# zijieli-Jlee/Temporal-Pointcloud-Upsampling-GAN

Hardware: AMD Instinct MI355X
Metric: GAN train-steps/sec (G+D) on 4096-pt x3-frame clips (higher is better)
Workload: dtype bf16; 1 GPU; cfg2: 4096-pt x3-frame fluid clips, full G+D adversarial step (SRNet(3,128) + FluidTempoDis(3) + FluidSpatialDis, Adam), all-keep mask regime, gate open, even iteration; batch 8 per GPU; per_gpu_batch=8, global_batch=8, parallelism=dp1, step_mode=hipgraph (1 graph per step)

## Files before the change

include/tpgan_ops.h:

```cpp
#ifndef TPGAN_OPS_H
#define TPGAN_OPS_H

#include <stddef.h>
#include <stdint.h>

#ifdef __cplusplus
extern "C" {
#endif

typedef enum {
    TPG_OK = 0,
    TPG_ERR_ARG = -1,
    TPG_ERR_LAUNCH = -2,
    TPG_ERR_UNSUPPORTED = -3
} tpg_status;

#define TPG_MAX_K 64

const char *tpg_version(void);
const char *tpg_target_arch(void);

int tpg_knn_f32(const float *p1, const float *p2, const int64_t *len1,
                const int64_t *len2, int B, int P1, int P2, int D, int K,
                float r2, float *dist, int64_t *idx, void *stream);

int tpg_knn_grid_f32(const float *p1, const float *p2, const int64_t *len1, const int64_t *len2, int B,
                     int P1, int P2, int K, float *dist, int64_t *idx, void *ws, void *stream);

int tpg_knn_mfma_f32(const float *p1, const float *p2, const int64_t *len1,
                     const int64_t *len2, int B, int P1, int P2, int D, int K,
                     float *dist, int64_t *idx, int redo, void *stream);

size_t tpg_frnn_grid_workspace_bytes(int B, int P2);
int tpg_frnn_grid_f32(const float *p1, const float *p2, const int64_t *len1, const int64_t *len2, int B, int P1,
                      int P2, int K, float r, float *dist, int64_t *idx, void *ws, void *stream);

int tpg_chamfer_fwd_f32(const float *src, const float *tgt, int B, int N, int M,
                        float *d1, int64_t *i1, float *d2, int64_t *i2,
                        void *stream);
size_t tpg_chamfer_bwd_workspace_bytes(int B, int N, int M);
int tpg_chamfer_bwd_f32(const float *src, const float *tgt, int B, int N, int M,
                        const int64_t *i1, const int64_t *i2, const float *g1,
                        const float *g2, float *gsrc, float *gtgt, void *ws, void *stream);

int tpg_fps_f32(const float *xyz, int B, int N, int m, float *temp, int32_t *idx,
                void *stream);

int tpg_fps_prefix_f32(const float *xyz, int B, int N, int m, float *temp, int32_t *idx,
                       const int32_t *prefix_in, int32_t *prefix_out, void *stream);

int tpg_fps_start_f32(const float *xyz, const int32_t *start, int skip_origin, int B, int N, int m,
                      float *temp, int32_t *idx, void *stream);

int tpg_gather_fwd_f32(const float *feat, const int32_t *idx, int B, int C, int N,
                       int S, float *out, void *stream);
int tpg_gather_bwd_f32(const float *gout, const int32_t *idx, int B, int C, int N,
                       int S, float *gfeat, void *stream);

int tpg_gather_rows_fwd_f32(const float *rows, const int32_t *idx, int B, int N, int S, int C, float *out, void *stream);
int tpg_gather_rows_bwd_f32(const float *gout, const int32_t *idx, int B, int N, int S, int C, float *grows,
                            void *stream);

int tpg_ball_query_f32(const float *xyz, const float *new_xyz, int B, int N, int S,
                       float radius, int nsample, int32_t *idx, void *stream);

int tpg_group_fwd_f32(const float *feat, const int32_t *idx, int B, int C, int N,
                      int S, int K, float *out, void *stream);
int tpg_group_bwd_f32(const float *gout, const int32_t *idx, int B, int C, int N,
                      int S, int K, float *gfeat, void *stream);

int tpg_three_nn_f32(const float *unknown, const float *known, int B, int n, int m,
                     float *dist2, int32_t *idx, void *stream);
int tpg_three_interp_fwd_f32(const float *feat, const int32_t *idx, const float *w,
                             int B, int C, int m, int n, float *out, void *stream);
int tpg_three_interp_bwd_f32(const float *gout, const int32_t *idx, const float *w,
                             int B, int C, int m, int n, float *gfeat,
                             void *stream);

typedef enum { TPG_DTYPE_F32 = 0, TPG_DTYPE_BF16 = 1 } tpg_dtype;

int tpg_rowcombine_fwd(const void *U, const void *QE, const int32_t *idx, int mode, int dtype_in,
                       int dtype_out, int B, int N, int S, int K, int C, float slope, void *out,
                       void *stream);

int tpg_invert_index(const int32_t *idx, int B, int N, int SK, int32_t *offs, int32_t *list,
                     int32_t *tmp, void *stream);

int tpg_rowcombine_bwd(const void *gout, const int32_t *idx, const int32_t *offs, const int32_t *list,
                       const void *E, int mode, int dtype_in, int dtype_out, int B, int N, int S, int K,
                       int C, float slope, void *gU, void *gQE, void *stream);

int tpg_rowcombine_edge_fwd(const void *Y, const int32_t *idx, int dtype_in, int dtype_out, int B, int N, int K, int C,
                            float slope_a, float slope_e, void *out, void *stream);
int tpg_rowcombine_edge_bwd(const void *gout, const int32_t *idx, const int32_t *offs, const int32_t *list,
                            const void *Y, int dtype_in, int dtype_out, int B, int N, int K, int C, float slope_a,
                            float slope_e, void *gY, void *stream);

int tpg_head_bn_act_fwd(const float *h, int B, int C, const float *gamma, const float *beta, float *running_mean,
                        float *running_var, long long *num_batches_tracked, float momentum, float eps, float slope,
                        const float *mask, float *y, float *mean, float *rstd, void *stream);
int tpg_head_bn_act_bwd(const float *gy, const float *h, const float *mean, const float *rstd, const float *gamma,
                        const float *beta, float slope, const float *mask, int B, int C, float *dh, float *dgamma,
                        float *dbeta, void *stream);

#define TPG_BN_PHASE_ALL 0
#define TPG_BN_PHASE_STATS 1
#define TPG_BN_PHASE_APPLY 2
size_t tpg_rowbn_workspace_bytes(int C, int nseg);
int tpg_rowbn_fwd(const void *x, int dtype_in, long long P, int K, int C, float eps, float momentum,
                  int training, float *running_mean, float *running_var, long long *num_batches_tracked,
                  const float *mean_shift, const float *gamma, const float *beta, float slope, float *mean,
                  float *rstd, void *y,
                  int dtype_out, uint8_t *argmax, void *ws, int nseg, int phase, void *stream);
int tpg_rowbn_bwd(const void *gy, int dtype_g, const void *x, int dtype_in, const uint8_t *argmax,
// ... 170 lines not shown
```

temporal-pointcloud-upsampling-gan_amd/_lib.py:

```python
import ctypes as C
import os

_HERE = os.path.dirname(os.path.abspath(__file__))
LIB_PATH = os.environ.get("TPGAN_HIP_LIBRARY") or os.path.join(_HERE, "csrc", "libtpgan_hip.so")

_P = C.c_void_p
_I = C.c_int
_F = C.c_float
_L = C.c_longlong

SIGNATURES = {
    "tpg_knn_f32": [_P, _P, _P, _P, _I, _I, _I, _I, _I, _F, _P, _P, _P],
    "tpg_knn_mfma_f32": [_P, _P, _P, _P, _I, _I, _I, _I, _I, _P, _P, _I, _P],
    "tpg_knn_grid_f32": [_P, _P, _P, _P, _I, _I, _I, _I, _P, _P, _P, _P],
    "tpg_frnn_grid_f32": [_P, _P, _P, _P, _I, _I, _I, _I, _F, _P, _P, _P, _P],
    "tpg_chamfer_fwd_f32": [_P, _P, _I, _I, _I, _P, _P, _P, _P, _P],
    "tpg_chamfer_bwd_f32": [_P, _P, _I, _I, _I, _P, _P, _P, _P, _P, _P, _P, _P],
    "tpg_fps_f32": [_P, _I, _I, _I, _P, _P, _P],
    "tpg_fps_prefix_f32": [_P, _I, _I, _I, _P, _P, _P, _P, _P],
    "tpg_fps_start_f32": [_P, _P, _I, _I, _I, _I, _P, _P, _P],
    "tpg_gather_fwd_f32": [_P, _P, _I, _I, _I, _I, _P, _P],
    "tpg_gather_bwd_f32": [_P, _P, _I, _I, _I, _I, _P, _P],
    "tpg_ball_query_f32": [_P, _P, _I, _I, _I, _F, _I, _P, _P],
    "tpg_group_fwd_f32": [_P, _P, _I, _I, _I, _I, _I, _P, _P],
    "tpg_group_bwd_f32": [_P, _P, _I, _I, _I, _I, _I, _P, _P],
    "tpg_three_nn_f32": [_P, _P, _I, _I, _I, _P, _P, _P],
    "tpg_three_interp_fwd_f32": [_P, _P, _P, _I, _I, _I, _I, _P, _P],
    "tpg_three_interp_bwd_f32": [_P, _P, _P, _I, _I, _I, _I, _P, _P],
    "tpg_gather_rows_fwd_f32": [_P, _P, _I, _I, _I, _I, _P, _P],
    "tpg_gather_rows_bwd_f32": [_P, _P, _I, _I, _I, _I, _P, _P],
    "tpg_rowcombine_fwd": [_P, _P, _P, _I, _I, _I, _I, _I, _I, _I, _I, _F, _P, _P],
    "tpg_invert_index": [_P, _I, _I, _I, _P, _P, _P, _P],
    "tpg_rowcombine_bwd": [_P, _P, _P, _P, _P, _I, _I, _I, _I, _I, _I, _I, _I, _F, _P, _P, _P],
    "tpg_rowcombine_edge_fwd": [_P, _P, _I, _I, _I, _I, _I, _I, _F, _F, _P, _P],
    "tpg_rowcombine_edge_bwd": [_P, _P, _P, _P, _P, _I, _I, _I, _I, _I, _I, _F, _F, _P, _P],
    "tpg_head_bn_act_fwd": [_P, _I, _I, _P, _P, _P, _P, _P, _F, _F, _F, _P, _P, _P, _P, _P],
    "tpg_head_bn_act_bwd": [_P, _P, _P, _P, _P, _P, _F, _P, _I, _I, _P, _P, _P, _P],
    "tpg_rowbn_fwd": [_P, _I, _L, _I, _I, _F, _F, _I, _P, _P, _P, _P, _P, _P, _F, _P, _P, _P, _I, _P, _P, _I, _I, _P],
    "tpg_rowbn_bwd": [_P, _I, _P, _I, _P, _P, _I, _L, _I, _I, _I, _P, _P, _P, _P, _F, _P, _P, _P, _P, _I, _I, _P],
    "tpg_cubic_interp_f32": [_P, _P, _P, _I, _I, _I, _I, _F, _P, _P, _P, _P],
    "tpg_spectral_norm_fwd": [_P, _P, _P, _I, _I, _I, _F, _P, _P, _P],
    "tpg_spectral_norm_bwd": [_P, _P, _P, _P, _P, _I, _I, _P, _P],
    "tpg_spectral_norm_multi_fwd": [_P, _I, _I, _P, _I, _F, _P],
    "tpg_spectral_norm_multi_fwd_split": [_P, _P, _I, _I, _P, _P, _L, _F, _P],
    "tpg_spectral_norm_multi_bwd": [_P, _I, _I, _P, _P, _P, _P, _P],
    "tpg_rowbn_bwd_sums": [_P, _I, _P, _I, _P, _P, _I, _L, _I, _I, _I, _P, _P, _P, _P, _F, _P, _P, _P, _P, _I, _P],
    "tpg_rowbn_bwd_sums_consts": [_P, _I, _P, _I, _P, _P, _I, _L, _I, _I, _I, _P, _P, _P, _P, _F, _P, _P, _P, _P, _P, _P, _I, _P],
    "tpg_rowbn_stats_consts": [_P, _I, _L, _I, _F, _F, _P, _P, _P, _P, _P, _P, _P, _P, _P, _P, _I, _P],
    "tpg_mlp_consts": [_P, _P, _P, _P, _P, _I, _I, _P, _P, _P],
    "tpg_mlp_max_prep": [_P, _P, _P, _F, _L, _I, _I, _P, _P],
    "tpg_mlp_dgrad": [_P, _P, _P, _I, _P, _P, _P, _F, _P, _I, _L, _I, _I, _I, _I, _P, _P, _P, _P, _P, _P, _P],
    "tpg_mlp_wgrad": [_P, _P, _P, _I, _P, _P, _P, _F, _L, _I, _I, _I, _I, _P, _P, _P],
    "tpg_mlp_bn_bwd_apply": [_P, _P, _P, _P, _L, _I, _I, _P, _P],
    "tpg_mlp_bn_bwd_apply_rowsum": [_P, _P, _P, _P, _L, _I, _I, _I, _P, _P, _P],
    "tpg_small_tail_fwd": [_P, _I, _P, _P, _F, _F, _L, _I, _I, _I, _I, _P, _P, _P],
    "tpg_small_tail_bwd": [_P, _P, _P, _P, _I, _P, _P, _F, _F, _L, _I, _I, _I, _I, _P, _P, _P, _P, _P],
    "tpg_rowlinear_fwd": [_P, _I, _P, _P, _L, _I, _I, _I, _F, _P, _I, _P],
    "tpg_rowlinear_dgrad": [_P, _P, _I, _P, _L, _I, _I, _I, _F, _P, _I, _P],
    "tpg_rowlinear_wgrad": [_P, _I, _P, _P, _I, _L, _I, _I, _I, _F, _P, _P, _P, _P],
    "tpg_mlp_fwd": [_P, _L, _I, _I, _I, _P, _I, _F, _P, _I, _P, _F, _F, _P, _P, _P, _P, _P, _P, _P, _P, _P, _P, _P],
    "tpg_mlp_infer_fwd": [_P, _P, _P, _I, _I, _I, _I, _I, _I, _I, _I, _P, _P, _P, _P, _P, _P, _F, _F, _F, _P, _P],
    "tpg_context_expand_f32": [_P, _P, _P, _I, _I, _I, _I, _P, _P, _P, _P, _P],
    "tpg_radius_reduce_f32": [_P, _P, _P, _P, _I, _I, _I, _F, _I, _P, _P, _P, _P],
    "tpg_radius_reduce_exhaustive_f32": [_P, _P, _P, _P, _I, _I, _I, _F, _I, _P, _P, _P],
    "tpg_patch_select_f32": [_P, _L, _P, _P, _P, _I, _I, _P, _P, _P],
    "tpg_clip_gather_high_f32": [_P, _P, _L, _P, _P, _P, _I, _P, _P, _I, _I, _I, _P, _P, _P],
    "tpg_clip_gather_low_f32": [_P, _P, _P, _F, _P, _L, _P, _P, _I, _I, _I, _I, _P, _P, _P],
    "tpg_frame_subset": [_P, _P, _I, _I, _P, _P],
    "tpg_action_gather_f32": [_P, _L, _P, _P, _P, _P, _I, _I, _I, _I, _P, _P, _P],
    "tpg_replace_dummy_centres": [_P, _P, _P, _I, _I, _I, _I, _P, _P, _P, _P],
    "tpg_emd_init_f32": [_P, _I, _I, _I, _I, _P, _P, _P],
    "tpg_emd_rounds_f32": [_P, _I, _I, _F, _F, _I, _I, _I, _I, _I, _P, _P, _P],
    "tpg_emd_finish_f32": [_P, _I, _I, _P, _P, _P, _P, _P, _P],
    "tpg_gaussian_row_sums_f32": [_P, _P, _P, _P, _I, _I, _I, _F, _P, _P],
    "tpg_render_points_f32": [_P, _P, _P, _I, _I, _P, _I, _I, _I, _I, _F, _F, _P, _P, _P, _P, _P, _P],
    "tpg_render_spheres_f32": [_P, _P, _I, _I, _P, _I, _I, _I, _F, _P, _P, _P, _P],
    "tpg_surface_smooth_f32": [_P, _I, _I, _I, _I, _F, _P, _P],
    "tpg_surface_shade_f32": [_P, _P, _P, _I, _I, _P, _I, _I, _I, _F, _F, _P, _P, _P, _P, _P],
    "tpg_pbf_predict_f32": [_P, _P, _P, _P, _I, _I, _F, _F, _P, _P, _P, _P],
    "tpg_pbf_grid_f32": [_P, _P, _I, _I, _F, _P, _P],
    "tpg_pbf_lambda_f32": [_P, _P, _I, _I, _F, _F, _F, _P, _P, _P, _P],
    "tpg_pbf_dp_f32": [_P, _P, _P, _P, _I, _I, _F, _F, _F, _F, _F, _P, _P, _P, _P],
    "tpg_pbf_finish_f32": [_P, _P, _P, _I, _I, _F, _F, _F, _P, _P, _P, _P],
    "tpg_iso_count_f32": [_P, _I, _I, _I, _F, _P, _P, _P],
    "tpg_iso_emit_f32": [_P, _I, _I, _I, _P, _F, _F, _P, _L, _L, _P, _P, _P, _P],
}
SIZE_GETTERS = ("tpg_rowbn_workspace_bytes", "tpg_mlp_workspace_bytes", "tpg_context_expand_workspace_bytes",
                "tpg_emd_workspace_bytes", "tpg_pbf_workspace_bytes", "tpg_iso_workspace_bytes")
OTHER_GETTERS = ("tpg_spectral_norm_multi_stride", "tpg_spectral_norm_multi_bwd_scratch",
                 "tpg_mlp_wgrad_workspace_bytes", "tpg_frnn_grid_workspace_bytes", "tpg_small_tail_workspace_bytes",
                 "tpg_chamfer_bwd_workspace_bytes", "tpg_rowlinear_wgrad_workspace_bytes", "tpg_rowlinear_supported",
                 "tpg_spectral_norm_split_rows", "tpg_spectral_norm_split_max_cn", "tpg_spectral_norm_split_max_rows",
                 "tpg_patch_select_workspace_bytes", "tpg_patch_select_max_k", "tpg_mlp_infer_supported")
STRING_GETTERS = ("tpg_version", "tpg_target_arch")

STATUS = {0: "TPG_OK", -1: "TPG_ERR_ARG", -2: "TPG_ERR_LAUNCH", -3: "TPG_ERR_UNSUPPORTED"}
# ... 59 lines not shown
```

temporal-pointcloud-upsampling-gan_amd/csrc/knn.hip:

```cpp
#include <cstdlib>
#include <type_traits>

#include <hip/hip_bf16.h>

#include "invert_index.hpp"
#include "knn_select.hpp"
#include "tpg_common.hpp"

namespace {

constexpr int KNN_WAVES = 4;

template <int D_T>
__device__ __forceinline__ float knn_dist(const float *__restrict__ qs,
                                          const float *__restrict__ c, int D) {
    float acc = 0.0f;
    if constexpr (D_T == 3) {
        acc = tpg_sq3(qs[0], qs[1], qs[2], c[0], c[1], c[2]);
    } else if constexpr (D_T > 0) {
        static_assert(D_T % 4 == 0, "vector path needs D % 4 == 0");
        const float4 *c4 = reinterpret_cast<const float4 *>(c);
        const float4 *q4 = reinterpret_cast<const float4 *>(qs);
#pragma unroll
        for (int d = 0; d < D_T / 4; ++d) {
// ... 152 lines not shown
        if (i >= P1 || lane >= K) continue;
        const size_t o = ((size_t)b * P1 + i) * K + lane;
        if (i >= n1 || n2 <= 0 || best[qq] == TPG_KNN_INF) { dist[o] = pad_d; idx[o] = pad_i; }
        else { dist[o] = tpg_knn_key_dist(best[qq]); idx[o] = tpg_knn_key_idx(best[qq]); }
    }
}

template <int D_T>
__global__ __launch_bounds__(KNN_WAVES * 64) void knn_redo_kernel(
    const float *__restrict__ p1, const float *__restrict__ p2, const int64_t *__restrict__ len1,
    const int64_t *__restrict__ len2, int P1, int P2, int K, float *__restrict__ dist, int64_t *__restrict__ idx) {
    __shared__ __attribute__((aligned(16))) float qs[D_T];
    __shared__ tpg_u64 slots[KNN_WAVES * 64];
    __shared__ tpg_u64 lists[KNN_WAVES * 64];
    const int lane = threadIdx.x & 63;
    const int wave = __builtin_amdgcn_readfirstlane(threadIdx.x >> 6);
    const int b = blockIdx.y;
    const int n1 = len1 ? (int)len1[b] : P1;
    const int n2 = len2 ? min((int)len2[b], P2) : P2;
    const float *cbase = p2 + (size_t)b * P2 * D_T;
    for (int u = 0; u < KNN_WAVES; ++u) {
        const int i = blockIdx.x * KNN_WAVES + u;
        if (i >= P1) break;
        const size_t q = (size_t)b * P1 + i;
        if (idx[q * K] != KM_REDO_MARK) continue;
        __syncthreads();
        if (threadIdx.x < D_T) qs[threadIdx.x] = p1[q * D_T + threadIdx.x];
        __syncthreads();
        tpg_u64 best = TPG_KNN_INF, thr = TPG_KNN_INF;
        if (i < n1)
            for (int base = wave * 64; base < n2; base += KNN_WAVES * 64) {
                const int j = base + lane;
                const tpg_u64 key =
                    j < n2 ? tpg_knn_key(knn_dist<D_T>(qs, cbase + (size_t)j * D_T, D_T), j) : TPG_KNN_INF;
                tpg_knn_merge(best, thr, key, K, lane, slots + wave * 64);
            }
        lists[wave * 64 + lane] = lane < K ? best : TPG_KNN_INF;
        __syncthreads();
        if (wave == 0) {
            best = TPG_KNN_INF;
            thr = TPG_KNN_INF;
            for (int w = 0; w < KNN_WAVES; ++w) tpg_knn_merge(best, thr, lists[w * 64 + lane], K, lane, slots);
            if (lane < K) {
                if (best == TPG_KNN_INF) { dist[q * K + lane] = 0.0f; idx[q * K + lane] = 0; }
                else { dist[q * K + lane] = tpg_knn_key_dist(best); idx[q * K + lane] = tpg_knn_key_idx(best); }
            }
        }
    }
}

#include "knn_mfma.hpp"

#ifndef TPG_KNN_MFMA_MIN_POINTS
#define TPG_KNN_MFMA_MIN_POINTS 2048
#endif

template <int D_T, int M>
int knn_mfma_launch_m(const float *p1, const float *p2, const int64_t *len1, const int64_t *len2, int B, int P1, int P2,
                      int K, float *dist, int64_t *idx, bool redo, hipStream_t st) {
    if (!tpg_allow_dynamic_lds<&knn_mfma_kernel<D_T, M>>((int)km_smem_bytes<D_T>())) return TPG_ERR_LAUNCH;
    const int gx = (P1 + KM_Q - 1) / KM_Q;
    const long long total = (long long)gx * B;
    if (total > (1ll << 30)) return TPG_ERR_ARG;
    const unsigned grid = (unsigned)((total + 7) / 8 * 8);
    hipLaunchKernelGGL((knn_mfma_kernel<D_T, M>), dim3(grid), dim3(KM_WAVES * 64), km_smem_bytes<D_T>(), st, p1, p2, len1, len2,
                       P1, P2, K, gx, (int)total, dist, idx);
    TPG_RETURN_IF_LAUNCH_FAILED();
    if (redo) {
        const dim3 rg((unsigned)((P1 + KNN_WAVES - 1) / KNN_WAVES), (unsigned)B);
        hipLaunchKernelGGL((knn_redo_kernel<D_T>), rg, dim3(KNN_WAVES * 64), 0, st, p1, p2, len1, len2, P1, P2, K, dist, idx);
        TPG_RETURN_IF_LAUNCH_FAILED();
    }
    return TPG_OK;
}

template <int D_T>
int knn_mfma_launch(const float *p1, const float *p2, const int64_t *len1, const int64_t *len2, int B, int P1, int P2,
                    int K, float *dist, int64_t *idx, bool redo, hipStream_t st) {
    if (K <= 12 && P2 < 16384) return knn_mfma_launch_m<D_T, 10>(p1, p2, len1, len2, B, P1, P2, K, dist, idx, redo, st);
    if (K <= 20 && P2 < 16384) return knn_mfma_launch_m<D_T, 14>(p1, p2, len1, len2, B, P1, P2, K, dist, idx, redo, st);
    return knn_mfma_launch_m<D_T, 16>(p1, p2, len1, len2, B, P1, P2, K, dist, idx, redo, st);
}

template <bool RADIUS>
int knn_launch(const float *p1, const float *p2, const int64_t *len1, const int64_t *len2, int B,
               int P1, int P2, int D, int K, float r2, float *dist, int64_t *idx,
               hipStream_t st) {
    if (B == 0 || P1 == 0) return TPG_OK;
    if (B > 65535) return TPG_ERR_ARG;
    const dim3 grid((unsigned)((P1 + KNN_WAVES - 1) / KNN_WAVES), (unsigned)B), block(KNN_WAVES * 64);
    const size_t smem = sizeof(float) * KNN_WAVES * ((D + 3) & ~3);
    if (smem > 64 * 1024) return TPG_ERR_UNSUPPORTED;
    const bool al = ((reinterpret_cast<uintptr_t>(p1) | reinterpret_cast<uintptr_t>(p2)) & 15) == 0;
#ifndef TPG_KNN_NO_MFMA
    static const bool mfma_on = [] { const char *e = getenv("TPG_KNN_MFMA"); return !(e && e[0] == '0'); }();
    if (mfma_on && !RADIUS && al && K > 1 && K <= KM_MAX_K && (D == 32 || D == 64) && P2 >= TPG_KNN_MFMA_MIN_POINTS) {
        if (D == 32) return knn_mfma_launch<32>(p1, p2, len1, len2, B, P1, P2, K, dist, idx, true, st);
        return knn_mfma_launch<64>(p1, p2, len1, len2, B, P1, P2, K, dist, idx, true, st);
    }
#endif
#ifndef TPG_KNN_NO_TILE
#ifdef TPG_KNN_TILE_Q
    constexpr int Q64 = TPG_KNN_TILE_Q, Q32 = TPG_KNN_TILE_Q;
    const bool tile32 = true;
#else
    constexpr int Q64 = 4, Q32 = 2;
    const bool tile32 = K <= 24;
#endif
    if (al && K > 1 && ((D == 64 && P1 >= KNN_WAVES * Q64) || (D == 32 && tile32 && P1 >= KNN_WAVES * Q32))) {
        if (D == 32) {
            const dim3 tg((unsigned)((P1 + KNN_WAVES * Q32 - 1) / (KNN_WAVES * Q32)), (unsigned)B);
            hipLaunchKernelGGL((knn_tile_kernel<32, Q32, RADIUS>), tg, block, 0, st, p1, p2, len1, len2, P1, P2, K, r2,
                               dist, idx);
        } else {
            const dim3 tg((unsigned)((P1 + KNN_WAVES * Q64 - 1) / (KNN_WAVES * Q64)), (unsigned)B);
            hipLaunchKernelGGL((knn_tile_kernel<64, Q64, RADIUS>), tg, block, 0, st, p1, p2, len1, len2, P1, P2, K, r2,
                               dist, idx);
        }
        TPG_RETURN_IF_LAUNCH_FAILED();
        return TPG_OK;
    }
#endif
#define TPG_KNN_GO(DT) \
    hipLaunchKernelGGL((knn_kernel<DT, RADIUS>), grid, block, smem, st, p1, p2, len1, len2, B, P1, \
                       P2, D, K, r2, dist, idx)
    if (D == 3) TPG_KNN_GO(3);
    else if (D == 32 && al) TPG_KNN_GO(32);
    else if (D == 64 && al) TPG_KNN_GO(64);
    else TPG_KNN_GO(0);
#undef TPG_KNN_GO
    TPG_RETURN_IF_LAUNCH_FAILED();
    return TPG_OK;
}

template <bool OWN_FIRST>
__global__ __launch_bounds__(256) void chamfer_bwd_gather_kernel(
    const float *__restrict__ a, const float *__restrict__ bcloud, int B, int N, int M,
    const int64_t *__restrict__ nn, const float *__restrict__ g, const int32_t *__restrict__ offs,
    const int32_t *__restrict__ list, const float *__restrict__ g2, float *__restrict__ ga) {
    const long long t = (long long)blockIdx.x * blockDim.x + threadIdx.x;
    if (t >= (long long)B * N) return;
    const int b = (int)(t / N), i = (int)(t - (long long)b * N);
    long long j = nn[t];
    j = j < 0 ? 0 : (j >= M ? M - 1 : j);
    const float gg = 2.0f * g[t];
    const float *pa = a + (size_t)t * 3;
    const float *pb = bcloud + ((size_t)b * M + j) * 3;
    const float ax = pa[0], ay = pa[1], az = pa[2];
    float acc[3] = {0.0f, 0.0f, 0.0f};
    const float own[3] = {gg * (ax - pb[0]), gg * (ay - pb[1]), gg * (az - pb[2])};
    if (OWN_FIRST) { acc[0] += own[0]; acc[1] += own[1]; acc[2] += own[2]; }
    const int32_t *of = offs + (size_t)b * (N + 1);
    const int32_t *ls = list + (size_t)b * M;
    const int p1 = of[i + 1];
    for (int p = of[i]; p < p1; ++p) {
        const int e = ls[p];
        const float h = 2.0f * g2[(size_t)b * M + e];
        const float *q = bcloud + ((size_t)b * M + e) * 3;
        acc[0] -= h * (q[0] - ax);
        acc[1] -= h * (q[1] - ay);
        acc[2] -= h * (q[2] - az);
    }
    if (!OWN_FIRST) { acc[0] += own[0]; acc[1] += own[1]; acc[2] += own[2]; }
    float *oa = ga + (size_t)t * 3;
    oa[0] = acc[0]; oa[1] = acc[1]; oa[2] = acc[2];
}

}

extern "C" int tpg_knn_f32(const float *p1, const float *p2, const int64_t *len1,
                           const int64_t *len2, int B, int P1, int P2, int D, int K, float r2,
                           float *dist, int64_t *idx, void *stream) {
    if (B < 0 || P1 < 0 || P2 < 0 || D <= 0 || K <= 0) return TPG_ERR_ARG;
    if (K > TPG_MAX_K) return TPG_ERR_UNSUPPORTED;
    if ((long long)B * P1 == 0) return TPG_OK;
    if (!p1 || !dist || !idx || (P2 > 0 && !p2)) return TPG_ERR_ARG;
    if (r2 >= 0.0f)
        return knn_launch<true>(p1, p2, len1, len2, B, P1, P2, D, K, r2, dist, idx, tpg_stream(stream));
    return knn_launch<false>(p1, p2, len1, len2, B, P1, P2, D, K, r2, dist, idx, tpg_stream(stream));
}

extern "C" int tpg_knn_mfma_f32(const float *p1, const float *p2, const int64_t *len1, const int64_t *len2, int B, int P1,
                                int P2, int D, int K, float *dist, int64_t *idx, int redo, void *stream) {
    if (B < 0 || P1 < 0 || P2 < 0 || K <= 1) return TPG_ERR_ARG;
    if ((D != 32 && D != 64) || K > KM_MAX_K) return TPG_ERR_UNSUPPORTED;
    if ((long long)B * P1 == 0) return TPG_OK;
    if (!p1 || !p2 || !dist || !idx || B > 65535) return TPG_ERR_ARG;
    if ((reinterpret_cast<uintptr_t>(p1) | reinterpret_cast<uintptr_t>(p2)) & 15) return TPG_ERR_ARG;
    if (D == 32) return knn_mfma_launch<32>(p1, p2, len1, len2, B, P1, P2, K, dist, idx, redo != 0, tpg_stream(stream));
    return knn_mfma_launch<64>(p1, p2, len1, len2, B, P1, P2, K, dist, idx, redo != 0, tpg_stream(stream));
}

extern "C" int tpg_chamfer_fwd_f32(const float *src, const float *tgt, int B, int N, int M,
                                   float *d1, int64_t *i1, float *d2, int64_t *i2, void *stream) {
    if (B < 0 || N <= 0 || M <= 0) return TPG_ERR_ARG;
    if (B == 0) return TPG_OK;
    if (!src || !tgt || !d1 || !i1 || !d2 || !i2) return TPG_ERR_ARG;
    int rc = knn_launch<false>(src, tgt, nullptr, nullptr, B, N, M, 3, 1, -1.0f, d1, i1, tpg_stream(stream));
    if (rc) return rc;
    return knn_launch<false>(tgt, src, nullptr, nullptr, B, M, N, 3, 1, -1.0f, d2, i2, tpg_stream(stream));
}

extern "C" size_t tpg_chamfer_bwd_workspace_bytes(int B, int N, int M) {
    if (B <= 0 || N <= 0 || M <= 0) return 0;
    return sizeof(int32_t) * ((size_t)B * ((size_t)N + 1 + 2 * (size_t)M) + (size_t)B * ((size_t)M + 1 + 2 * (size_t)N)) + 64;
}

extern "C" int tpg_chamfer_bwd_f32(const float *src, const float *tgt, int B, int N, int M,
                                   const int64_t *i1, const int64_t *i2, const float *g1,
                                   const float *g2, float *gsrc, float *gtgt, void *ws, void *stream) {
    if (B < 0 || N <= 0 || M <= 0) return TPG_ERR_ARG;
    if (B == 0) return TPG_OK;
    if (!src || !tgt || !i1 || !i2 || !g1 || !g2 || !gsrc || !gtgt || !ws) return TPG_ERR_ARG;
    hipStream_t st = tpg_stream(stream);
    int32_t *offs_s = static_cast<int32_t *>(ws);
    int32_t *list_s = offs_s + (size_t)B * (N + 1);
    int32_t *tmp_s = list_s + (size_t)B * M;
    int32_t *offs_t = tmp_s + (size_t)B * M;
    int32_t *list_t = offs_t + (size_t)B * (M + 1);
    int32_t *tmp_t = list_t + (size_t)B * N;
    int rc = tpg_inv::launch<int64_t>(i2, B, N, M, offs_s, list_s, tmp_s, st);
    if (rc) return rc;
    rc = tpg_inv::launch<int64_t>(i1, B, M, N, offs_t, list_t, tmp_t, st);
    if (rc) return rc;
    const long long t1 = (long long)B * N, t2 = (long long)B * M;
    hipLaunchKernelGGL(chamfer_bwd_gather_kernel<true>, dim3((unsigned)((t1 + 255) / 256)), dim3(256), 0, st, src,
                       tgt, B, N, M, i1, g1, offs_s, list_s, g2, gsrc);
    hipLaunchKernelGGL(chamfer_bwd_gather_kernel<false>, dim3((unsigned)((t2 + 255) / 256)), dim3(256), 0, st, tgt,
                       src, B, M, N, i2, g2, offs_t, list_t, g1, gtgt);
    TPG_RETURN_IF_LAUNCH_FAILED();
    return TPG_OK;
}
```

temporal-pointcloud-upsampling-gan_amd/ops.py:

```python
import ctypes as C

import os

import numpy as np
import torch

from . import _lib

_BACKENDS = {}


class OpTimer:

    def __init__(self):
        self.pending = {}

    def record(self, name, nbytes, stream_of, launch, flops=0):
        st = torch.cuda.current_stream(stream_of.device)
        a = torch.cuda.Event(enable_timing=True)
        b = torch.cuda.Event(enable_timing=True)
        a.record(st)
        out = launch()
        b.record(st)
        self.pending.setdefault(name, []).append((a, b, nbytes, flops))
# ... 62 lines not shown
        self.idx = t.device.index
        self.prev = None

    def __enter__(self):
        cur = torch.cuda.current_device()
        if self.idx is not None and cur != self.idx:
            self.prev = cur
            torch.cuda.set_device(self.idx)

    def __exit__(self, *a):
        if self.prev is not None:
            torch.cuda.set_device(self.prev)


class HipBackend:

    name = "hip"

    def __init__(self):
        self.lib = _lib.load()
        self._ws = {}
        self._ws_retired = []
        self._sn_plans = {}

    def _retire(self, ws):
        if ws is not None:
            self._ws_retired.append(ws)

    def _workspace(self, kind, ref, need, dtype=torch.float32, zeroed=False):
        key = (kind, ref.device, torch.cuda.current_stream(ref.device).cuda_stream)
        ws = self._ws.get(key)
        if ws is None or ws.numel() < need:
            self._retire(ws)
            ws = (torch.zeros if zeroed else torch.empty)(need, dtype=dtype, device=ref.device)
            self._ws[key] = ws
        return ws

    def _call(self, symbol, op, nbytes, ref, *args, flops=0):
        fn = getattr(self.lib, symbol)
        with _DeviceGuard(ref):
            _lib.check(_run(op, nbytes, ref, lambda: fn(*args, _stream(ref)), flops), symbol)

    GRID_MIN_POINTS = 1024
    GRID_MIN_PAIRS = 6.0e7

    KNN_GRID_MIN_POINTS = 2048
    CHAMFER_GRID_MIN_POINTS = 8192

    def _grid_ws(self, ref, B, P2):
        return self._workspace("frnn", ref, self.lib.tpg_frnn_grid_workspace_bytes(B, P2), dtype=torch.uint8)

    def knn(self, p1, p2, len1, len2, K, r2, r=None):
        B, P1, D = p1.shape
        P2 = p2.shape[1]
        dist = torch.empty((B, P1, K), dtype=torch.float32, device=p1.device)
        idx = torch.empty((B, P1, K), dtype=torch.int64, device=p1.device)
        if (r is not None and r2 is not None and D == 3 and K <= 64 and P2 >= self.GRID_MIN_POINTS
                and float(B) * P1 * P2 >= self.GRID_MIN_PAIRS and float(r) > 0):
            self._call("tpg_frnn_grid_f32", "frnn_grid", 4 * B * D * (P1 + P2) + 12 * B * P1 * K, p1,
                       _ptr(p1), _ptr(p2), _ptr(len1), _ptr(len2), B, P1, P2, K, float(np.float32(r)), _ptr(dist),
                       _ptr(idx), _ptr(self._grid_ws(p1, B, P2)))
            return dist, idx
        if (r2 is None and D == 3 and K <= 64 and P2 >= self.KNN_GRID_MIN_POINTS
                and float(B) * P1 * P2 >= self.GRID_MIN_PAIRS):
            self._call("tpg_knn_grid_f32", "knn_grid", 4 * B * D * (P1 + P2) + 12 * B * P1 * K, p1,
                       _ptr(p1), _ptr(p2), _ptr(len1), _ptr(len2), B, P1, P2, K, _ptr(dist), _ptr(idx),
                       _ptr(self._grid_ws(p1, B, P2)))
            return dist, idx
        mfma = r2 is None and D in (32, 64) and 1 < K <= 24 and P2 >= 2048 and os.environ.get("TPG_KNN_MFMA", "1")[:1] != "0"
        self._call("tpg_knn_f32", "knn_mfma" if mfma else "knn", 4 * B * D * (P1 + P2) + 12 * B * P1 * K, p1,
                   _ptr(p1), _ptr(p2), _ptr(len1), _ptr(len2), B, P1, P2, D, K,
                   -1.0 if r2 is None else r2, _ptr(dist), _ptr(idx), flops=12.0 * B * P1 * P2 * D if mfma else 0)
        return dist, idx

    def knn_mfma(self, p1, p2, len1, len2, K, redo=True):
        B, P1, D = p1.shape
        P2 = p2.shape[1]
        dist = torch.zeros((B, P1, K), dtype=torch.float32, device=p1.device)
        idx = torch.zeros((B, P1, K), dtype=torch.int64, device=p1.device)
        self._call("tpg_knn_mfma_f32", "knn_mfma", 4 * B * D * (P1 + P2) + 12 * B * P1 * K, p1,
                   _ptr(p1), _ptr(p2), _ptr(len1), _ptr(len2), B, P1, P2, D, K, _ptr(dist), _ptr(idx), 1 if redo else 0,
                   flops=12.0 * B * P1 * P2 * D)

        return dist, idx

    def cubic_interp(self, query, pos, field, cutoff):
        B, Nq, _ = query.shape
        Np, F_ = pos.shape[1], field.shape[2]
        plain = torch.empty((B, Nq, F_), dtype=torch.float32, device=query.device)
        pad = torch.empty_like(plain)
        hits = torch.empty((B, Nq), dtype=torch.int32, device=query.device)
        self._call("tpg_cubic_interp_f32", "cubic_interp", 12 * B * (Nq + Np) + 4 * B * Np * F_ + 8 * B * Nq * F_,
                   query, _ptr(query), _ptr(pos), _ptr(field), B, Nq, Np, F_, float(cutoff), _ptr(plain),
                   _ptr(pad), _ptr(hits))
        return plain, pad, hits

    def radius_reduce(self, query, pos, lenq, lenp, r, kernel, want_count=True, want_sum=True, grid=None):
        B, Nq, _ = query.shape
        Np = pos.shape[1]
        count = torch.empty((B, Nq), dtype=torch.int32, device=query.device) if want_count else None
        total = torch.empty((B, Nq), dtype=torch.float32, device=query.device) if want_sum else None
        if grid is None:
            grid = Np >= self.GRID_MIN_POINTS and float(B) * Nq * Np >= self.GRID_MIN_PAIRS
        nbytes = 12 * B * (Nq + Np) + 4 * B * Nq * (int(want_count) + int(want_sum))
        args = (_ptr(query), _ptr(pos), _ptr(lenq), _ptr(lenp), B, Nq, Np, float(np.float32(r)), int(kernel),
                _ptr(count), _ptr(total))
        if grid and B > 0 and Nq > 0 and Np > 0:
            self._call("tpg_radius_reduce_f32", "radius_reduce_grid", nbytes, query, *args,
                       _ptr(self._grid_ws(query, B, Np)))
        else:
            self._call("tpg_radius_reduce_exhaustive_f32", "radius_reduce", nbytes, query, *args)
        return count, total

    EMD_NARROW_WORK = 256 * 1024
    EMD_NARROW_MIN = 16
    EMD_CHECK_EVERY = 8
    EMD_NARROW_ROUNDS = 256

    def emd_narrow_at(self, n):
        return max(0, min(n, max(self.EMD_NARROW_MIN, self.EMD_NARROW_WORK // max(n, 1))))

    def emd_begin(self, xyz1, xyz2, phases):
        B, n, _ = xyz1.shape
        dev = xyz1.device
        st = {"xyz1": xyz1, "B": B, "n": n, "phases": int(phases),
              "dist": torch.empty((B, n), dtype=torch.float32, device=dev),
              "assignment": torch.empty((B, n), dtype=torch.int32, device=dev),
              "price": torch.empty((B, n), dtype=torch.float32, device=dev),
              "rounds": torch.zeros((B,), dtype=torch.int32, device=dev)}
        st["ws"] = self._workspace("emd", xyz1, self.lib.tpg_emd_workspace_bytes(B, n), dtype=torch.uint8)
        self._call("tpg_emd_init_f32", "emd_init", 16 * B * n, xyz1, _ptr(xyz2), B, n, xyz2.shape[1], int(phases),
                   _ptr(st["assignment"]), _ptr(st["ws"]))
        return st

    def emd_batch(self, st, eps, iters, scaling, narrow_at, wide):
        B, n = st["B"], st["n"]
        self._call("tpg_emd_rounds_f32", "emd_rounds", 16 * B * n, st["xyz1"], _ptr(st["xyz1"]), B, n, float(eps),
                   float(scaling), st["phases"], int(iters), int(wide), self.EMD_NARROW_ROUNDS, int(narrow_at),
                   _ptr(st["assignment"]), _ptr(st["ws"]))
        launches = (2 * int(wide) if narrow_at < n else 0) + (1 if narrow_at > 0 else 0)
        return st["ws"][:32 * B].view(torch.int32).view(B, 8).cpu(), launches

    def emd_end(self, st):
        B, n = st["B"], st["n"]
        self._call("tpg_emd_finish_f32", "emd_finish", 16 * B * n, st["xyz1"], _ptr(st["xyz1"]), B, n,
                   _ptr(st["assignment"]), _ptr(st["ws"]), _ptr(st["dist"]), _ptr(st["price"]), _ptr(st["rounds"]))
        return st["dist"], st["assignment"], st["price"], st["rounds"]

    def emd_match(self, xyz1, xyz2, eps, iters, phases, scaling, narrow_at=None, check_every=None):
        B, n, _ = xyz1.shape
        if B == 0 or n == 0:
            dev = xyz1.device
            return (torch.empty((B, n), dtype=torch.float32, device=dev),
                    torch.empty((B, n), dtype=torch.int32, device=dev),
                    torch.empty((B, n), dtype=torch.float32, device=dev),
                    torch.zeros((B,), dtype=torch.int32, device=dev))
        narrow_at = self.emd_narrow_at(n) if narrow_at is None else max(0, min(int(narrow_at), n))
        wide = self.EMD_CHECK_EVERY if check_every is None else int(check_every)
        st = self.emd_begin(xyz1, xyz2, phases)
        while True:
            rec, _ = self.emd_batch(st, eps, iters, scaling, narrow_at, wide)
            status = rec[:, 3]
            if bool((status == 2).any()):
                b = int(torch.nonzero(status == 2)[0])
                raise RuntimeError(f"emd_match: cloud {b} still has {int(rec[b, 2])} unassigned persons after "
                                   f"{int(rec[b, 1])} rounds (iters = {int(iters)})")
# ... 2511 lines not shown
```

Baseline: 80.45 steps/s.

## Add LDS-resident MFMA kNN kernel for feature-space queries on small point sets

Adds a kNN kernel for D=32/64 features with 512-1024 candidate points. It computes the full query-by-candidate distance block with split-bf16 MFMA into LDS, picks a per-query threshold from per-lane minima with an error bound, then collects candidates and re-ranks them exactly in fp32. Queries where that fails fall back to a redo kernel. It is routed automatically when the existing MFMA path's minimum point count is not met, replacing the tiled scalar kernel for those sizes, at the cost of large dynamic LDS use and lower occupancy.

Measured after the change: 82.41 steps/s (median of 6 runs). +2.4%, better.

```diff
diff --git a/include/tpgan_ops.h b/include/tpgan_ops.h
--- a/include/tpgan_ops.h
+++ b/include/tpgan_ops.h
@@ -30,6 +30,10 @@
 int tpg_knn_mfma_f32(const float *p1, const float *p2, const int64_t *len1,
                      const int64_t *len2, int B, int P1, int P2, int D, int K,
                      float *dist, int64_t *idx, int redo, void *stream);
+
+int tpg_knn_small_f32(const float *p1, const float *p2, const int64_t *len1,
+                      const int64_t *len2, int B, int P1, int P2, int D, int K,
+                      float *dist, int64_t *idx, int redo, void *stream);
 
 size_t tpg_frnn_grid_workspace_bytes(int B, int P2);
 int tpg_frnn_grid_f32(const float *p1, const float *p2, const int64_t *len1, const int64_t *len2, int B, int P1,
diff --git a/temporal-pointcloud-upsampling-gan_amd/_lib.py b/temporal-pointcloud-upsampling-gan_amd/_lib.py
--- a/temporal-pointcloud-upsampling-gan_amd/_lib.py
+++ b/temporal-pointcloud-upsampling-gan_amd/_lib.py
@@ -12,6 +12,7 @@
 SIGNATURES = {
     "tpg_knn_f32": [_P, _P, _P, _P, _I, _I, _I, _I, _I, _F, _P, _P, _P],
     "tpg_knn_mfma_f32": [_P, _P, _P, _P, _I, _I, _I, _I, _I, _P, _P, _I, _P],
+    "tpg_knn_small_f32": [_P, _P, _P, _P, _I, _I, _I, _I, _I, _P, _P, _I, _P],
     "tpg_knn_grid_f32": [_P, _P, _P, _P, _I, _I, _I, _I, _P, _P, _P, _P],
     "tpg_frnn_grid_f32": [_P, _P, _P, _P, _I, _I, _I, _I, _F, _P, _P, _P, _P],
     "tpg_chamfer_fwd_f32": [_P, _P, _I, _I, _I, _P, _P, _P, _P, _P],
diff --git a/temporal-pointcloud-upsampling-gan_amd/csrc/knn.hip b/temporal-pointcloud-upsampling-gan_amd/csrc/knn.hip
--- a/temporal-pointcloud-upsampling-gan_amd/csrc/knn.hip
+++ b/temporal-pointcloud-upsampling-gan_amd/csrc/knn.hip
@@ -258,6 +258,35 @@
     return knn_mfma_launch_m<D_T, 16>(p1, p2, len1, len2, B, P1, P2, K, dist, idx, redo, st);
 }
 
+#include "knn_small.hpp"
+
+#ifndef TPG_KNN_SMALL_MIN_POINTS
+#define TPG_KNN_SMALL_MIN_POINTS 512
+#endif
+#ifndef TPG_KNN_SMALL_MAX_POINTS
+#define TPG_KNN_SMALL_MAX_POINTS 1025
+#endif
+static_assert(TPG_KNN_SMALL_MAX_POINTS <= KS_MAX_P2 + 1, "the distance matrix of knn_small_kernel must fit the LDS");
+
+template <int D_T>
+int knn_small_launch(const float *p1, const float *p2, const int64_t *len1, const int64_t *len2, int B, int P1, int P2,
+                     int K, float *dist, int64_t *idx, bool redo, hipStream_t st) {
+    if (P2 > KS_MAX_P2) return TPG_ERR_UNSUPPORTED;
+    if (!tpg_allow_dynamic_lds<&knn_small_kernel<D_T>>((int)ks_smem_bytes<D_T>(KS_MAX_P2))) return TPG_ERR_LAUNCH;
+    const int gx = (P1 + KS_Q - 1) / KS_Q;
+    const long long total = (long long)gx * B;
+    if (total > (1ll << 30)) return TPG_ERR_ARG;
+    hipLaunchKernelGGL((knn_small_kernel<D_T>), dim3((unsigned)total), dim3(KS_WAVES * 64), ks_smem_bytes<D_T>(P2), st, p1, p2,
+                       len1, len2, P1, P2, K, gx, dist, idx);
+    TPG_RETURN_IF_LAUNCH_FAILED();
+    if (redo) {
+        const dim3 rg((unsigned)((P1 + KNN_WAVES - 1) / KNN_WAVES), (unsigned)B);
+        hipLaunchKernelGGL((knn_redo_kernel<D_T>), rg, dim3(KNN_WAVES * 64), 0, st, p1, p2, len1, len2, P1, P2, K, dist, idx);
+        TPG_RETURN_IF_LAUNCH_FAILED();
+    }
+    return TPG_OK;
+}
+
 template <bool RADIUS>
 int knn_launch(const float *p1, const float *p2, const int64_t *len1, const int64_t *len2, int B,
                int P1, int P2, int D, int K, float r2, float *dist, int64_t *idx,
@@ -273,6 +302,14 @@
     if (mfma_on && !RADIUS && al && K > 1 && K <= KM_MAX_K && (D == 32 || D == 64) && P2 >= TPG_KNN_MFMA_MIN_POINTS) {
         if (D == 32) return knn_mfma_launch<32>(p1, p2, len1, len2, B, P1, P2, K, dist, idx, true, st);
         return knn_mfma_launch<64>(p1, p2, len1, len2, B, P1, P2, K, dist, idx, true, st);
+    }
+#endif
+#ifndef TPG_KNN_NO_SMALL
+    static const bool small_on = [] { const char *e = getenv("TPG_KNN_SMALL"); return !(e && e[0] == '0'); }();
+    if (small_on && !RADIUS && al && K > 1 && K <= KM_MAX_K && (D == 32 || D == 64) && P2 >= TPG_KNN_SMALL_MIN_POINTS &&
+        P2 < TPG_KNN_SMALL_MAX_POINTS) {
+        if (D == 32) return knn_small_launch<32>(p1, p2, len1, len2, B, P1, P2, K, dist, idx, true, st);
+        return knn_small_launch<64>(p1, p2, len1, len2, B, P1, P2, K, dist, idx, true, st);
     }
 #endif
 #ifndef TPG_KNN_NO_TILE
@@ -367,6 +404,17 @@
     return knn_mfma_launch<64>(p1, p2, len1, len2, B, P1, P2, K, dist, idx, redo != 0, tpg_stream(stream));
 }
 
+extern "C" int tpg_knn_small_f32(const float *p1, const float *p2, const int64_t *len1, const int64_t *len2, int B, int P1,
+                                 int P2, int D, int K, float *dist, int64_t *idx, int redo, void *stream) {
+    if (B < 0 || P1 < 0 || P2 < 0 || K <= 1) return TPG_ERR_ARG;
+    if ((D != 32 && D != 64) || K > KM_MAX_K || P2 > KS_MAX_P2) return TPG_ERR_UNSUPPORTED;
+    if ((long long)B * P1 == 0) return TPG_OK;
+    if (!p1 || !p2 || !dist || !idx || B > 65535) return TPG_ERR_ARG;
+    if ((reinterpret_cast<uintptr_t>(p1) | reinterpret_cast<uintptr_t>(p2)) & 15) return TPG_ERR_ARG;
+    if (D == 32) return knn_small_launch<32>(p1, p2, len1, len2, B, P1, P2, K, dist, idx, redo != 0, tpg_stream(stream));
+    return knn_small_launch<64>(p1, p2, len1, len2, B, P1, P2, K, dist, idx, redo != 0, tpg_stream(stream));
+}
+
 extern "C" int tpg_chamfer_fwd_f32(const float *src, const float *tgt, int B, int N, int M,
                                    float *d1, int64_t *i1, float *d2, int64_t *i2, void *stream) {
     if (B < 0 || N <= 0 || M <= 0) return TPG_ERR_ARG;
diff --git a/temporal-pointcloud-upsampling-gan_amd/csrc/knn_small.hpp b/temporal-pointcloud-upsampling-gan_amd/csrc/knn_small.hpp
--- /dev/null
+++ b/temporal-pointcloud-upsampling-gan_amd/csrc/knn_small.hpp
@@ -0,0 +1,270 @@
+#pragma once
+
+constexpr int KS_Q = 32;
+constexpr int KS_WAVES = 8;
+constexpr int KS_QW = KS_Q / KS_WAVES;
+constexpr int KS_MIN_VALID = 64;
+constexpr int KS_MAX_P2 = 1024;
+static_assert(KS_Q % KS_WAVES == 0 && KS_QW % 2 == 0 && KS_MAX_P2 <= 65536, "queries per wave in pairs; 16-bit candidate slots");
+
+constexpr int ks_ldq(int P2) { return ((P2 + 31) & ~31) + 4; }
+template <int D_T>
+constexpr size_t ks_smem_bytes(int P2) {
+    return sizeof(float) * ((size_t)KS_Q * ks_ldq(P2) + D_T + KS_Q + KS_WAVES * D_T) + sizeof(tpg_u64) * KS_WAVES * 64 +
+           sizeof(int) * (KS_Q + 2) + sizeof(unsigned short) * KS_Q * KM_CAP;
+}
+
+template <int D_T>
+__global__ __launch_bounds__(KS_WAVES * 64, 4) void knn_small_kernel(
+    const float *__restrict__ p1, const float *__restrict__ p2, const int64_t *__restrict__ len1,
+    const int64_t *__restrict__ len2, int P1, int P2, int K, int gx, float *__restrict__ dist, int64_t *__restrict__ idx) {
+    constexpr int KS = D_T / 16;
+    constexpr int NV = 2 * KS;
+    constexpr int G = KS_WAVES * 64 / D_T;
+    constexpr int RG = km_tile_rows<D_T>() / G;
+    constexpr int V4 = D_T / 4;
+    static_assert(RG * G == km_tile_rows<D_T>() && G * D_T == KS_WAVES * 64, "origin: one (group, dim) per thread");
+    extern __shared__ __attribute__((aligned(16))) unsigned char ks_smem[];
+    const int LDQ = ks_ldq(P2);
+    float *dm = reinterpret_cast<float *>(ks_smem);
+    float *org = dm + KS_Q * LDQ;
+    float *nqs = org + D_T;
+    float *qrow = nqs + KS_Q;
+    tpg_u64 *keys = reinterpret_cast<tpg_u64 *>(qrow + KS_WAVES * D_T);
+    int *cnt = reinterpret_cast<int *>(keys + KS_WAVES * 64);
+    unsigned *pmax = reinterpret_cast<unsigned *>(cnt + KS_Q);
+    unsigned short *cbuf = reinterpret_cast<unsigned short *>(pmax + 2);
+
+    const int b = blockIdx.x / gx;
+    const int q0 = (blockIdx.x - b * gx) * KS_Q;
+    const int tid = threadIdx.x, lane = tid & 63;
+    const int wave = __builtin_amdgcn_readfirstlane(tid >> 6);
+    const int c = lane & 31, h = lane >> 5;
+    const int n1 = len1 ? (int)len1[b] : P1;
+    const int n2 = len2 ? min((int)len2[b], P2) : P2;
+    float *od = dist + (size_t)b * P1 * K;
+    int64_t *oi = idx + (size_t)b * P1 * K;
+    if (n2 < KS_MIN_VALID) {
+        if (tid < KS_Q && q0 + tid < P1) oi[(size_t)(q0 + tid) * K] = KM_REDO;
+        return;
+    }
+    const float *cb = p2 + (size_t)b * P2 * D_T;
+
+    {
+        const int d = tid % D_T, g = tid / D_T;
+        const int rows0 = min(n2, km_tile_rows<D_T>());
+        float a = 0.0f;
+#pragma unroll
+        for (int r = 0; r < RG; ++r)
+            if (g * RG + r < rows0) a += cb[(size_t)(g * RG + r) * D_T + d];
+        dm[g * D_T + d] = a;
+        if (tid == 0) *pmax = 0u;
+        __syncthreads();
+        if (tid < D_T) {
+            float s = 0.0f;
+#pragma unroll
+            for (int gg = 0; gg < G; ++gg) s += dm[gg * D_T + tid];
+            org[tid] = s / (float)rows0;
+        }
+        __syncthreads();
+    }
+
+    auto load_half = [&](const float *row, bool valid, float4 (&x)[NV]) {
+#pragma unroll
+        for (int i = 0; i < NV; ++i)
+            x[i] = valid ? *reinterpret_cast<const float4 *>(row + 16 * (i >> 1) + 8 * h + 4 * (i & 1)) : make_float4(0.f, 0.f, 0.f, 0.f);
+    };
+    auto centre_split = [&](const float4 (&x)[NV], bool valid, float scale, uint4 (&hi)[KS], uint4 (&lo)[KS]) {
+        float s = 0.0f;
+#pragma unroll
+        for (int ks = 0; ks < KS; ++ks) {
+            float y[8];
+#pragma unroll
+            for (int v = 0; v < 2; ++v) {
+                float4 t = make_float4(0.f, 0.f, 0.f, 0.f);
+                const float4 o = *reinterpret_cast<const float4 *>(org + 16 * ks + 8 * h + 4 * v);
+                if (valid) { t.x = x[2 * ks + v].x - o.x; t.y = x[2 * ks + v].y - o.y; t.z = x[2 * ks + v].z - o.z; t.w = x[2 * ks + v].w - o.w; }
+                y[4 * v] = t.x; y[4 * v + 1] = t.y; y[4 * v + 2] = t.z; y[4 * v + 3] = t.w;
+                s += t.x * t.x + t.y * t.y + t.z * t.z + t.w * t.w;
+            }
+            km_split2(scale * y[0], scale * y[1], hi[ks].x, lo[ks].x);
+            km_split2(scale * y[2], scale * y[3], hi[ks].y, lo[ks].y);
+            km_split2(scale * y[4], scale * y[5], hi[ks].z, lo[ks].z);
+            km_split2(scale * y[6], scale * y[7], hi[ks].w, lo[ks].w);
+        }
+        return s + __shfl_xor(s, 32);
+    };
+
+    uint4 bqh[KS], bql[KS];
+    {
+        const int qi = q0 + c;
+        float4 x[NV];
+        load_half(p1 + ((size_t)b * P1 + (qi < P1 ? qi : 0)) * D_T, qi < P1, x);
+        const float nq = centre_split(x, qi < P1, 1.0f, bqh, bql);
+        if (tid < KS_Q) nqs[tid] = nq;
+    }
+
+    const uint4 ones = h == 0 ? make_uint4(0x3f803f80u, 0x00003f80u, 0u, 0u) : make_uint4(0u, 0u, 0u, 0u);
+    const km_f32x16 zero16 = {0.f, 0.f, 0.f, 0.f, 0.f, 0.f, 0.f, 0.f, 0.f, 0.f, 0.f, 0.f, 0.f, 0.f, 0.f, 0.f};
+    const int NS = (n2 + 31) >> 5;
+    float mymax = 0.0f;
+    for (int s = wave; s < NS; s += KS_WAVES) {
+        const bool valid = 32 * s + c < n2;
+        float4 cur[NV];
+        load_half(cb + (size_t)min(32 * s + c, n2 - 1) * D_T, valid, cur);
+        uint4 ah[KS], al[KS];
+        const float ss = centre_split(cur, valid, -2.0f, ah, al);
+        const float nv = valid ? ss : KM_BIG;
+        const __hip_bfloat16 t0 = __float2bfloat16(nv);
+        const float r0 = nv - __bfloat162float(t0);
+        const __hip_bfloat16 t1 = __float2bfloat16(r0);
+        const __hip_bfloat16 t2 = __float2bfloat16(r0 - __bfloat162float(t1));
+        const unsigned w0 = (unsigned)*reinterpret_cast<const unsigned short *>(&t0) |
+                            ((unsigned)*reinterpret_cast<const unsigned short *>(&t1) << 16);
+        const unsigned w1 = (unsigned)*reinterpret_cast<const unsigned short *>(&t2);
+        const uint4 an = h == 0 ? make_uint4(w0, w1, 0u, 0u) : make_uint4(0u, 0u, 0u, 0u);
+        if (valid) mymax = (ss > mymax || ss != ss) ? ss : mymax;
+        km_f32x16 acc = __builtin_amdgcn_mfma_f32_32x32x16_bf16(__builtin_bit_cast(km_bf16x8, an), __builtin_bit_cast(km_bf16x8, ones), zero16, 0, 0, 0);
+#pragma unroll
+        for (int ks = 0; ks < KS; ++ks) {
+            const km_bf16x8 Ah = __builtin_bit_cast(km_bf16x8, ah[ks]), Al = __builtin_bit_cast(km_bf16x8, al[ks]);
+            const km_bf16x8 Bh = __builtin_bit_cast(km_bf16x8, bqh[ks]), Bl = __builtin_bit_cast(km_bf16x8, bql[ks]);
+            acc = __builtin_amdgcn_mfma_f32_32x32x16_bf16(Al, Bh, acc, 0, 0, 0);
+            acc = __builtin_amdgcn_mfma_f32_32x32x16_bf16(Ah, Bl, acc, 0, 0, 0);
+            acc = __builtin_amdgcn_mfma_f32_32x32x16_bf16(Ah, Bh, acc, 0, 0, 0);
+        }
+        float *drow = dm + c * LDQ + 32 * s + 4 * h;
+#pragma unroll
+        for (int g = 0; g < 4; ++g)
+            *reinterpret_cast<float4 *>(drow + 8 * g) = make_float4(acc[4 * g], acc[4 * g + 1], acc[4 * g + 2], acc[4 * g + 3]);
+    }
+    atomicMax(pmax, __float_as_uint(mymax));
+    __syncthreads();
+
+    const float sq_pmax = sqrtf(__uint_as_float(*pmax));
+    constexpr float C1 = 1.220703125e-4f;
+    constexpr float C2 = (float)(8 * D_T + 64) * 5.9604644775390625e-8f;
+    const int NT = (n2 + 63) >> 6;
+    for (int qq = 0; qq < KS_QW; ++qq) {
+        const int ql = wave * KS_QW + qq, i = q0 + ql;
+        if (i >= P1 || i >= n1) continue;
+        const float *drow = dm + ql * LDQ;
+        float mn = KM_BIG;
+        for (int t = 0; t < NT; t += 4) {
+            float v[4];
+#pragma unroll
+            for (int u = 0; u < 4; ++u) { const int j = 64 * (t + u) + lane; v[u] = j < n2 ? drow[j] : KM_BIG; }
+            mn = fminf(fminf(mn, v[0]), fminf(fminf(v[1], v[2]), v[3]));
+        }
+        int rank = 0;
+#pragma unroll 8
+        for (int s = 0; s < 64; ++s) {
+            const float o = __uint_as_float((unsigned)__builtin_amdgcn_readlane((int)__float_as_uint(mn), s));
+            rank += (o < mn || (o == mn && s < lane)) ? 1 : 0;
+        }
+        const tpg_u64 at = __ballot(rank == K - 1);
+        const float T = __uint_as_float((unsigned)__builtin_amdgcn_readlane(
+            (int)__float_as_uint(mn), __builtin_amdgcn_readfirstlane(at ? __builtin_ctzll(at) : 0)));
+        const float sqq = sqrtf(nqs[ql]);
+        const float eq = (C1 * sqq * sq_pmax + C2 * (sqq + sq_pmax) * (sqq + sq_pmax)) * 1.001f;
+        float thr = T + 2.0f * eq;
+        thr = thr + fabsf(thr) * 9.5367431640625e-7f;
+        int n = 0;
+        if (at != 0 && thr < 1.0e29f) {
+            for (int t = 0; t < NT; t += 4) {
+                float v[4];
+#pragma unroll
+                for (int u = 0; u < 4; ++u) { const int j = 64 * (t + u) + lane; v[u] = j < n2 ? drow[j] : KM_BIG; }
+#pragma unroll
+                for (int u = 0; u < 4; ++u) {
+                    const bool hit = v[u] <= thr;
+                    const tpg_u64 m = __ballot(hit);
+                    const int pos = n + (int)__builtin_amdgcn_mbcnt_hi((unsigned)(m >> 32), __builtin_amdgcn_mbcnt_lo((unsigned)m, 0u));
+                    if (hit && pos < KM_CAP) cbuf[ql * KM_CAP + pos] = (unsigned short)(64 * (t + u) + lane);
+                    n += __popcll(m);
+                }
+            }
+        } else {
+            n = KM_CAP + 1;
+        }
+        if (lane == 0) cnt[ql] = n;
+    }
+
+    float *qs = qrow + wave * D_T;
+    tpg_u64 *ks_ = keys + wave * 64;
+    const tpg_u64 INF = TPG_KNN_INF;
+    auto fetch = [&](int qq, float4 (&row)[V4], float &qx, int &j, int &n) {
+        const int ql = wave * KS_QW + qq, i = q0 + ql;
+        j = -1;
+        n = -1;
+        if (qq >= KS_QW || i >= P1 || i >= n1) return;
+        if (lane < D_T) qx = p1[((size_t)b * P1 + i) * D_T + lane];
+        n = cnt[ql];
+        if (n <= KM_CAP && lane < n) {
+            j = cbuf[ql * KM_CAP + lane];
+            const float4 *c4 = reinterpret_cast<const float4 *>(cb + (size_t)j * D_T);
+#pragma unroll
+            for (int d = 0; d < V4; ++d) row[d] = c4[d];
+        }
+    };
+    auto finish = [&](int qq, const float4 (&row)[V4], float qx, int j, int n) {
+        const int i = q0 + wave * KS_QW + qq;
+        if (qq >= KS_QW || i >= P1) return;
+        if (i >= n1) {
+            if (lane < K) { od[(size_t)i * K + lane] = 0.0f; oi[(size_t)i * K + lane] = 0; }
+            return;
+        }
+        if (lane < D_T) qs[lane] = qx;
+        tpg_u64 key = INF;
+        if (j >= 0) {
+            const float4 *q4 = reinterpret_cast<const float4 *>(qs);
+            float acc = 0.0f;
+#pragma unroll
+            for (int d = 0; d < V4; ++d) {
+                const float4 qv = q4[d];
+                float t;
+                t = qv.x - row[d].x; acc = acc + t * t;
+                t = qv.y - row[d].y; acc = acc + t * t;
+                t = qv.z - row[d].z; acc = acc + t * t;
+                t = qv.w - row[d].w; acc = acc + t * t;
+            }
+            key = tpg_knn_key(acc, j);
+        }
+        ks_[lane] = key;
+        const int nk = (n >= K && n <= KM_CAP) ? n : 0;
+        int rank = 0;
+        for (int s = 0; s < nk; s += 8)
+#pragma unroll
+            for (int u = 0; u < 8; ++u) rank += ks_[s + u] < key ? 1 : 0;
+        if (nk > 0) {
+            if (rank < K && key != INF) {
+                od[(size_t)i * K + rank] = tpg_knn_key_dist(key);
+                oi[(size_t)i * K + rank] = tpg_knn_key_idx(key);
+            }
+        } else if (lane == 0) {
+            oi[(size_t)i * K] = KM_REDO;
+        }
+    };
+    float4 rowA[V4];
+    float qA = 0.0f;
+    int jA, nA;
+    if constexpr (D_T == 32) {
+        float4 rowB[V4];
+        float qB = 0.0f;
+        int jB, nB;
+        fetch(0, rowA, qA, jA, nA);
+#pragma unroll 1
+        for (int qq = 0; qq < KS_QW; qq += 2) {
+            fetch(qq + 1, rowB, qB, jB, nB);
+            finish(qq, rowA, qA, jA, nA);
+            fetch(qq + 2, rowA, qA, jA, nA);
+            finish(qq + 1, rowB, qB, jB, nB);
+        }
+    } else {
+#pragma unroll 1
+        for (int qq = 0; qq < KS_QW; ++qq) {
+            fetch(qq, rowA, qA, jA, nA);
+            finish(qq, rowA, qA, jA, nA);
+        }
+    }
+}
diff --git a/temporal-pointcloud-upsampling-gan_amd/ops.py b/temporal-pointcloud-upsampling-gan_amd/ops.py
--- a/temporal-pointcloud-upsampling-gan_amd/ops.py
+++ b/temporal-pointcloud-upsampling-gan_amd/ops.py
@@ -168,6 +168,15 @@
                    _ptr(p1), _ptr(p2), _ptr(len1), _ptr(len2), B, P1, P2, D, K, _ptr(dist), _ptr(idx), 1 if redo else 0,
                    flops=12.0 * B * P1 * P2 * D)
 
+        return dist, idx
+
+    def knn_small(self, p1, p2, len1, len2, K, redo=True):
+        B, P1, D = p1.shape
+        P2 = p2.shape[1]
+        dist = torch.zeros((B, P1, K), dtype=torch.float32, device=p1.device)
+        idx = torch.zeros((B, P1, K), dtype=torch.int64, device=p1.device)
+        self._call("tpg_knn_small_f32", "knn", 4 * B * D * (P1 + P2) + 12 * B * P1 * K, p1,
+                   _ptr(p1), _ptr(p2), _ptr(len1), _ptr(len2), B, P1, P2, D, K, _ptr(dist), _ptr(idx), 1 if redo else 0)
         return dist, idx
 
     def cubic_interp(self, query, pos, field, cutoff):
```
